# equinor/gordo-components

Measured on NVIDIA H100. Metric: anomaly windows/sec (64-tag feedforward_hourglass AE, 1k machines x 10k rows per GPU, fused predict+score), higher is better.
Workload: dtype split tf32/bf16/fp16

## Files before the change

### gordo_components_b200/csrc/ffae_infer_tc.cu

```cuda
#include <atomic>
#include <cuda_bf16.h>
#include <cuda_fp16.h>
#include "gb_common.cuh"
#include "gb_sm90.cuh"

namespace {

using namespace gb::sm90;

constexpr int TILE = 64;
constexpr int NWG = 3;
constexpr int NTHREADS = 128 * NWG;
constexpr int MAXL = 8;
constexpr int W = 64;
constexpr int BOX_COLS = 32;
constexpr int BOX_BYTES = TILE * BOX_COLS * 4;
constexpr int TILE_BYTES = 2 * BOX_BYTES;
constexpr int STAGE_BYTES = 2 * TILE_BYTES * NWG;
constexpr int OBOX_ROWS = 16;
constexpr int OBOX_BYTES = OBOX_ROWS * BOX_COLS * 4;

struct TcArgs {
  CUtensorMap tm_x, tm_y;
  CUtensorMap tm_o[4];
  int T;
  int L;
  int N[MAXL], Np[MAXL], k16[MAXL];
  int img0_ofs[MAXL], img1_ofs[MAXL], img2_ofs[MAXL];
  int bias_ofs[MAXL];
  int pofs[MAXL];
  int K[MAXL];
  int w_bytes;
  int vec_ofs;
  int stage_ofs;
  int n_jobs, tiles_per_job;
  long pstride;
  const float* params;
  const gb_job* jobs;
  const float *y, *scale, *feat_thr, *agg_thr;
  float *o_model, *o_ts, *o_tu, *o_conf, *o_tots, *o_totu, *o_totconf;
  unsigned int* work_ctr;
};

constexpr float TANH_ARG_SCALE = 2.8853900817779268f;
__device__ __forceinline__ float tanh_from_scaled(float t) {
  float e, r;
  asm("ex2.approx.ftz.f32 %0, %1;" : "=f"(e) : "f"(t));
  asm("rcp.approx.ftz.f32 %0, %1;" : "=f"(r) : "f"(e + 1.0f));
  return fmaf(-2.0f, r, 1.0f);
}

__device__ __forceinline__ uint32_t pack_bf16(float lo, float hi) {
  const __nv_bfloat162 p = __floats2bfloat162_rn(lo, hi);
  return *reinterpret_cast<const uint32_t*>(&p);
}
__device__ __forceinline__ float trunc_tf32(float v) { return __uint_as_float(__float_as_uint(v) & 0xffffe000u); }
__device__ __forceinline__ void split_f16(float a0, float a1, uint32_t& w1, uint32_t& w2) {
  const __half2 h = __floats2half2_rn(a0, a1);
  const float2 f = __half22float2(h);
  const __half2 r = __floats2half2_rn(a0 - f.x, a1 - f.y);
  w1 = *reinterpret_cast<const uint32_t*>(&h);
  w2 = *reinterpret_cast<const uint32_t*>(&r);
}

__host__ __device__ __forceinline__ int tf32_row(int k) { return (k & ~7) | (((k & 7) >> 1) + 4 * (k & 1)); }

template <int N>
__device__ __forceinline__ void mma_layer0(float* d, const uint32_t (&xhi)[4][8], const uint32_t (&alo)[4][4], const uint32_t (&abf)[4][4],
                                           uint32_t img0, uint32_t img1, uint32_t img2, int k16) {
  const uint32_t lbo = N * 16, step = 2 * N * 16;
#pragma unroll
  for (int ks = 0; ks < 8; ++ks)
    if (ks < 2 * k16) {
      const uint32_t a[4] = {xhi[ks >> 1][4 * (ks & 1) + 0], xhi[ks >> 1][4 * (ks & 1) + 1], xhi[ks >> 1][4 * (ks & 1) + 2], xhi[ks >> 1][4 * (ks & 1) + 3]};
      if (N == 16) wgmma_rs_tf32_n16(d, a, desc_noswizzle(img0 + ks * step, lbo, 128), ks > 0);
      if (N == 32) wgmma_rs_tf32_n32(d, a, desc_noswizzle(img0 + ks * step, lbo, 128), ks > 0);
      if (N == 48) wgmma_rs_tf32_n48(d, a, desc_noswizzle(img0 + ks * step, lbo, 128), ks > 0);
      if (N == 64) wgmma_rs_tf32_n64(d, a, desc_noswizzle(img0 + ks * step, lbo, 128), ks > 0);
    }
#pragma unroll
  for (int ks = 0; ks < 4; ++ks)
    if (ks < k16) {
      if (N == 16) wgmma_rs_bf16_n16(d, alo[ks], desc_noswizzle(img1 + ks * step, lbo, 128), 1);
      if (N == 32) wgmma_rs_bf16_n32(d, alo[ks], desc_noswizzle(img1 + ks * step, lbo, 128), 1);
      if (N == 48) wgmma_rs_bf16_n48(d, alo[ks], desc_noswizzle(img1 + ks * step, lbo, 128), 1);
      if (N == 64) wgmma_rs_bf16_n64(d, alo[ks], desc_noswizzle(img1 + ks * step, lbo, 128), 1);
    }
#pragma unroll
  for (int ks = 0; ks < 4; ++ks)
    if (ks < k16) {
      if (N == 16) wgmma_rs_bf16_n16(d, abf[ks], desc_noswizzle(img2 + ks * step, lbo, 128), 1);
      if (N == 32) wgmma_rs_bf16_n32(d, abf[ks], desc_noswizzle(img2 + ks * step, lbo, 128), 1);
      if (N == 48) wgmma_rs_bf16_n48(d, abf[ks], desc_noswizzle(img2 + ks * step, lbo, 128), 1);
      if (N == 64) wgmma_rs_bf16_n64(d, abf[ks], desc_noswizzle(img2 + ks * step, lbo, 128), 1);
    }
}
template <int N>
__device__ __forceinline__ void mma_f16(float* d, const uint32_t* a, uint64_t desc, uint32_t acc) {
  if (N == 16) wgmma_rs_f16_n16(d, a, desc, acc);
  if (N == 32) wgmma_rs_f16_n32(d, a, desc, acc);
  if (N == 48) wgmma_rs_f16_n48(d, a, desc, acc);
  if (N == 64) wgmma_rs_f16_n64(d, a, desc, acc);
}
template <int N>
__device__ __forceinline__ void mma_hidden(float* d, const uint32_t (&a1)[4][4], const uint32_t (&a2)[4][4], uint32_t img0, uint32_t img1, int k16) {
  const uint32_t lbo = N * 16, step = 2 * N * 16;
#pragma unroll
  for (int ks = 0; ks < 4; ++ks)
    if (ks < k16) mma_f16<N>(d, a2[ks], desc_noswizzle(img0 + ks * step, lbo, 128), ks > 0);
#pragma unroll
  for (int ks = 0; ks < 4; ++ks)
    if (ks < k16) mma_f16<N>(d, a1[ks], desc_noswizzle(img1 + ks * step, lbo, 128), 1);
#pragma unroll
  for (int ks = 0; ks < 4; ++ks)
    if (ks < k16) mma_f16<N>(d, a1[ks], desc_noswizzle(img0 + ks * step, lbo, 128), 1);
}

__device__ __forceinline__ int box_ofs(int r, int col) { return r * 128 + (((col >> 2) ^ (r & 7)) << 4) + ((col & 3) << 2); }
__device__ __forceinline__ int tile_ofs(int r, int col) { return (col >> 5) * BOX_BYTES + box_ofs(r, col & 31); }

__device__ __forceinline__ void warpgroup_sync(int wg) { asm volatile("bar.sync %0, 128;" ::"r"(wg + 1) : "memory"); }

__device__ __forceinline__ void fence_acc(float (&d)[32]) {
#pragma unroll
  for (int i = 0; i < 32; ++i) fence_reg(d[i]);
}
template <int R, int C>
__device__ __forceinline__ void fence_frag(uint32_t (&f)[R][C]) {
#pragma unroll
  for (int i = 0; i < R; ++i)
#pragma unroll
    for (int j = 0; j < C; ++j) fence_reg(f[i][j]);
}

__global__ void __launch_bounds__(NTHREADS, 1) ffae_tc_kernel(const __grid_constant__ TcArgs a) {
  extern __shared__ __align__(1024) uint8_t smem[];
  const int tid = threadIdx.x, lane = tid & 31;
  const int warp = __shfl_sync(0xffffffffu, tid >> 5, 0);
  const int wg = warp >> 2, wq = warp & 3;
  const int g = lane >> 2, t = lane & 3;
  const uint32_t sbase = smem_u32(smem);
  const int TP = a.T, L = a.L;
  const bool has_y = a.y != nullptr;
  const bool totals = has_y && (a.o_tots || a.o_totu || a.o_totconf);
  const float inv_w = 1.0f / (float)TP;

  __shared__ __align__(8) unsigned long long s_bar[2 * NWG];
  const uint32_t stage = (sbase + a.stage_ofs + 1023) & ~1023u;
  const uint32_t xbuf = stage + wg * 2 * TILE_BYTES, ybuf = xbuf + TILE_BYTES;
  const uint8_t* xs = smem + (xbuf - sbase);
  const uint8_t* ys = smem + (ybuf - sbase);
  const uint32_t bar_x = smem_u32(&s_bar[wg]), bar_y = smem_u32(&s_bar[NWG + wg]);
  const bool leader = (tid & 127) == 0;
  uint32_t x_phase = 0, y_phase = 0;
  const uint32_t obox0 = ybuf + wq * OBOX_BYTES, obox1 = obox0 + BOX_BYTES;
  if (tid == 0) {
    for (int i = 0; i < 2 * NWG; ++i) mbar_init(smem_u32(&s_bar[i]), 1);
    asm volatile("fence.mbarrier_init.release.cluster;" ::: "memory");
  }

  __shared__ int s_item[3];
  __shared__ int s_range[2];
  if (tid == 0) s_range[0] = s_range[1] = 0;
  int cur_slot = -1;

  while (true) {
    if (tid == 0) {
      const int tpj = a.tiles_per_job, g_total = a.n_jobs * tpj;
      int gg = s_range[0], g_end = s_range[1];
      if (gg >= g_end) {
        const int seen = (int)*reinterpret_cast<volatile unsigned int*>(a.work_ctr);
        const int left = g_total - seen, per_cta = left / (int)gridDim.x;
        int size = per_cta * 2 >= 3 * tpj ? tpj : (per_cta >= tpj / 3 ? (tpj + 2) / 3 : (tpj + 5) / 6);
        if (size < 1) size = 1;
        if (seen % tpj != 0 && size > tpj - seen % tpj) size = tpj - seen % tpj;
        gg = (int)atomicAdd(a.work_ctr, (unsigned int)size);
        g_end = gg + size < g_total ? gg + size : g_total;
      }
      if (gg >= g_total) {
        s_item[0] = -1;
      } else {
        const int job_id = gg / tpj, tile_begin = gg - job_id * tpj;
        const int tile_end = min(tpj, tile_begin + (g_end - gg));
        s_item[0] = job_id; s_item[1] = tile_begin; s_item[2] = tile_end;
        gg += tile_end - tile_begin;
      }
      s_range[0] = gg; s_range[1] = g_end;
    }
    __syncthreads();
    const int job_id = s_item[0], tile_begin = s_item[1], tile_end = s_item[2];
    if (job_id < 0) break;
    const gb_job job = a.jobs[job_id];
    const int row_begin = tile_begin * TILE;
    if (row_begin >= job.n_rows) {
      __syncthreads();
      continue;
    }
    const int row_end = min(job.n_rows, tile_end * TILE);
    const int n_tiles = (row_end - row_begin + TILE - 1) / TILE;

    if (job.slot != cur_slot) {
      cur_slot = job.slot;
      const float* P = a.params + (long)job.slot * a.pstride;
      for (int i = tid; i < a.w_bytes / 16; i += NTHREADS) reinterpret_cast<uint4*>(smem)[i] = make_uint4(0, 0, 0, 0);
      __syncthreads();
      for (int l = 0; l < L; ++l) {
        const int K = a.K[l], N = a.N[l], Np = a.Np[l], KN = K * N;
        const float* Ws = P + a.pofs[l];
        for (int i = tid; i < KN; i += NTHREADS) {
          const int k = i / N, n = i - k * N;
          const float w = __ldg(Ws + i);
          const int i8 = ((k >> 3) * Np + n) * 8 + (k & 7);
          if (l == 0) {
            const float hi = __uint_as_float((__float_as_uint(w) + 0x1000u) & 0xffffe000u);
            const int kt = tf32_row(k);
            reinterpret_cast<float*>(smem + a.img0_ofs[0])[((kt >> 2) * Np + n) * 4 + (kt & 3)] = hi;
            reinterpret_cast<__nv_bfloat16*>(smem + a.img1_ofs[0])[i8] = __float2bfloat16_rn(hi);
            reinterpret_cast<__nv_bfloat16*>(smem + a.img2_ofs[0])[i8] = __float2bfloat16_rn(w - hi);
          } else {
            const __half w1 = __float2half_rn(w);
            reinterpret_cast<__half*>(smem + a.img0_ofs[l])[i8] = w1;
            reinterpret_cast<__half*>(smem + a.img1_ofs[l])[i8] = __float2half_rn(w - __half2float(w1));
          }
        }
        const float bscale = (l + 1 < L) ? TANH_ARG_SCALE : 1.0f;
        for (int n = tid; n < N; n += NTHREADS) reinterpret_cast<float*>(smem + a.bias_ofs[l])[n] = __ldg(Ws + KN + n) * bscale;
      }
      float* vec = reinterpret_cast<float*>(smem + a.vec_ofs);
      if (tid < W) {
        vec[tid] = (tid < TP && a.scale) ? __ldg(a.scale + (long)job.slot * TP + tid) : 0.f;
        vec[W + tid] = (tid < TP && a.feat_thr) ? 1.0f / __ldg(a.feat_thr + (long)job.slot * TP + tid) : 0.f;
      }
      fence_proxy_async();
    }
    __syncthreads();

    const float* vec = reinterpret_cast<const float*>(smem + a.vec_ofs);
    auto load_tile = [&](const CUtensorMap* m, uint32_t buf, uint32_t bar, int tt) {
      const int row = (int)(job.x_row + row_begin + tt * TILE);
      mbar_expect_tx(bar, TILE_BYTES);
      tma_load_2d(buf, m, 0, row, bar);
      tma_load_2d(buf + BOX_BYTES, m, BOX_COLS, row, bar);
    };
    if (leader && wg < n_tiles) load_tile(&a.tm_x, xbuf, bar_x, wg);
    for (int tt = wg; tt < n_tiles; tt += NWG) {
      float d[32];
      uint32_t a1[4][4] = {}, a2[4][4] = {};
      {
        float xr[2][16];
        mbar_wait(bar_x, x_phase);
        x_phase ^= 1;
#pragma unroll
        for (int hr = 0; hr < 2; ++hr)
#pragma unroll
          for (int c = 0; c < 8; ++c) {
            const float2 v = *reinterpret_cast<const float2*>(xs + tile_ofs(wq * 16 + g + 8 * hr, 8 * c + 2 * t));
            xr[hr][2 * c] = v.x;
            xr[hr][2 * c + 1] = v.y;
          }
        if (lane == 0) bulk_wait_read<0>();
        warpgroup_sync(wg);
        if (leader) {
          if (tt + NWG < n_tiles) load_tile(&a.tm_x, xbuf, bar_x, tt + NWG);
          if (has_y) load_tile(&a.tm_y, ybuf, bar_y, tt);
        }
        uint32_t xhi[4][8], alo[4][4], abf[4][4];
#pragma unroll
        for (int kk = 0; kk < 4; ++kk) {
#pragma unroll
          for (int hh = 0; hh < 2; ++hh) {
            xhi[kk][4 * hh + 0] = __float_as_uint(trunc_tf32(xr[0][4 * kk + 2 * hh]));
            xhi[kk][4 * hh + 1] = __float_as_uint(trunc_tf32(xr[1][4 * kk + 2 * hh]));
            xhi[kk][4 * hh + 2] = __float_as_uint(trunc_tf32(xr[0][4 * kk + 2 * hh + 1]));
            xhi[kk][4 * hh + 3] = __float_as_uint(trunc_tf32(xr[1][4 * kk + 2 * hh + 1]));
          }
#pragma unroll
          for (int q = 0; q < 4; ++q) {
            const float v0 = xr[q & 1][4 * kk + 2 * (q >> 1)], v1 = xr[q & 1][4 * kk + 2 * (q >> 1) + 1];
            alo[kk][q] = pack_bf16(v0 - trunc_tf32(v0), v1 - trunc_tf32(v1));
            abf[kk][q] = pack_bf16(v0, v1);
          }
        }
        const int k16 = a.k16[0];
        const uint32_t i0 = sbase + a.img0_ofs[0], i1 = sbase + a.img1_ofs[0], i2 = sbase + a.img2_ofs[0];
        wgmma_fence();
        switch (a.Np[0]) {
          case 16: mma_layer0<16>(d, xhi, alo, abf, i0, i1, i2, k16); break;
          case 32: mma_layer0<32>(d, xhi, alo, abf, i0, i1, i2, k16); break;
          case 48: mma_layer0<48>(d, xhi, alo, abf, i0, i1, i2, k16); break;
          default: mma_layer0<64>(d, xhi, alo, abf, i0, i1, i2, k16); break;
        }
        wgmma_commit();
        wgmma_wait<0>();
        fence_acc(d);
        fence_frag(xhi);
        fence_frag(alo);
        fence_frag(abf);
      }

      for (int l = 0; l < L; ++l) {
        if (l > 0) {
          const uint32_t i0 = sbase + a.img0_ofs[l], i1 = sbase + a.img1_ofs[l];
          const int k16 = a.k16[l];
          wgmma_fence();
          switch (a.Np[l]) {
            case 16: mma_hidden<16>(d, a1, a2, i0, i1, k16); break;
            case 32: mma_hidden<32>(d, a1, a2, i0, i1, k16); break;
            case 48: mma_hidden<48>(d, a1, a2, i0, i1, k16); break;
            default: mma_hidden<64>(d, a1, a2, i0, i1, k16); break;
          }
          wgmma_commit();
          wgmma_wait<0>();
          fence_acc(d);
          fence_frag(a1);
          fence_frag(a2);
        }
        if (l + 1 == L) break;
        const float* bl = reinterpret_cast<const float*>(smem + a.bias_ofs[l]);
        const int nt = a.Np[l] >> 3;
#pragma unroll
        for (int j = 0; j < 8; ++j) {
          if (j < nt) {
            const float2 b = *reinterpret_cast<const float2*>(bl + 8 * j + 2 * t);
            const float v0 = tanh_from_scaled(fmaf(d[4 * j], TANH_ARG_SCALE, b.x)), v1 = tanh_from_scaled(fmaf(d[4 * j + 1], TANH_ARG_SCALE, b.y));
            const float v2 = tanh_from_scaled(fmaf(d[4 * j + 2], TANH_ARG_SCALE, b.x)), v3 = tanh_from_scaled(fmaf(d[4 * j + 3], TANH_ARG_SCALE, b.y));
            split_f16(v0, v1, a1[j >> 1][2 * (j & 1)], a2[j >> 1][2 * (j & 1)]);
            split_f16(v2, v3, a1[j >> 1][2 * (j & 1) + 1], a2[j >> 1][2 * (j & 1) + 1]);
          }
        }
      }

      const float* bo = reinterpret_cast<const float*>(smem + a.bias_ofs[L - 1]);
      const int wrow = row_begin + tt * TILE + wq * 16;
      const int trow = wrow + g;
      const int nt = a.Np[L - 1] >> 3;
      float2 yr[2][8];
      if (has_y) {
        mbar_wait(bar_y, y_phase);
        y_phase ^= 1;
#pragma unroll
        for (int hr = 0; hr < 2; ++hr)
#pragma unroll
          for (int j = 0; j < 8; ++j) yr[hr][j] = *reinterpret_cast<const float2*>(ys + tile_ofs(wq * 16 + g + 8 * hr, 8 * j + 2 * t));
      }
      auto model_out = [&](int hr, int j) {
        const float2 b = *reinterpret_cast<const float2*>(bo + 8 * j + 2 * t);
        return j < nt ? make_float2(d[4 * j + 2 * hr] + b.x, d[4 * j + 2 * hr + 1] + b.y) : make_float2(0.f, 0.f);
      };

      const int n_live = min(row_end - wrow, OBOX_ROWS);
      if (n_live > 0) {
        int k = 0;
#pragma unroll
        for (int arr = 0; arr < 4; ++arr) {
          float* o = arr == 0 ? a.o_model : arr == 1 ? a.o_tu : arr == 2 ? a.o_ts : a.o_conf;
          if (o == nullptr || (arr > 0 && !has_y)) continue;
#pragma unroll
          for (int h = 0; h < 2; ++h) {
            if (h == 1 && TP <= BOX_COLS) break;
            const uint32_t box = (k & 1) ? obox1 : obox0;
            if (k >= 2 && lane == 0) bulk_wait_read<1>();
            __syncwarp();
            uint8_t* bs = smem + (box - sbase);
#pragma unroll
            for (int hr = 0; hr < 2; ++hr)
#pragma unroll
              for (int jj = 0; jj < 4; ++jj) {
                const int j = 4 * h + jj, col = 8 * j + 2 * t;
                float2 v = model_out(hr, j);
                if (arr > 0) {
                  const float2 yv = yr[hr][j];
                  v = make_float2(fabsf(v.x - yv.x), fabsf(v.y - yv.y));
                  const float2 s = *reinterpret_cast<const float2*>(vec + (arr == 3 ? W : 0) + col);
                  if (arr > 1) v = make_float2(v.x * s.x, v.y * s.y);
                }
                *reinterpret_cast<float2*>(bs + box_ofs(g + 8 * hr, 8 * jj + 2 * t)) = v;
              }
            fence_proxy_async();
            __syncwarp();
            if (n_live == OBOX_ROWS) {
              if (lane == 0) {
                tma_store_2d(&a.tm_o[arr], box, BOX_COLS * h, (int)(job.out_row + wrow));
                bulk_commit();
              }
            } else {
              const int cols = min(BOX_COLS, TP - BOX_COLS * h);
              for (int i = lane; i < n_live * 8; i += 32) {
                const int r = i >> 3, c = i & 7;
                if (4 * c < cols)
                  __stcs(reinterpret_cast<float4*>(o + (job.out_row + wrow + r) * (long)TP + BOX_COLS * h + 4 * c),
                         *reinterpret_cast<const float4*>(bs + box_ofs(r, 4 * c)));
              }
            }
            ++k;
          }
        }
      }
      if (totals) {
        float ss[2] = {0.f, 0.f}, su[2] = {0.f, 0.f};
#pragma unroll
        for (int hr = 0; hr < 2; ++hr)
#pragma unroll
          for (int j = 0; j < 8; ++j) {
            const int col = 8 * j + 2 * t;
            if (j < nt && col < TP) {
              const float2 yh = model_out(hr, j), yv = yr[hr][j];
              const float2 sc = *reinterpret_cast<const float2*>(vec + col);
              const float2 df = make_float2(fabsf(yh.x - yv.x), fabsf(yh.y - yv.y));
              const float2 e = make_float2(df.x * sc.x, df.y * sc.y);
              su[hr] += df.x * df.x + df.y * df.y;
              ss[hr] += e.x * e.x + e.y * e.y;
            }
          }
#pragma unroll
        for (int hr = 0; hr < 2; ++hr) {
          ss[hr] += __shfl_xor_sync(0xffffffffu, ss[hr], 1);
          ss[hr] += __shfl_xor_sync(0xffffffffu, ss[hr], 2);
          su[hr] += __shfl_xor_sync(0xffffffffu, su[hr], 1);
          su[hr] += __shfl_xor_sync(0xffffffffu, su[hr], 2);
          const int r = trow + 8 * hr;
          if (t == 0 && r < row_end) {
            const long go = job.out_row + r;
            const float ts_ = ss[hr] * inv_w, tu_ = su[hr] * inv_w;
            if (a.o_tots) a.o_tots[go] = ts_;
            if (a.o_totu) a.o_totu[go] = tu_;
            if (a.o_totconf) a.o_totconf[go] = ts_ / __ldg(a.agg_thr + job.slot);
          }
        }
      }
    }
    __syncthreads();
  }
  if (lane == 0) bulk_wait<0>();
}

constexpr int WORK_CTRS = 1024;
__device__ unsigned int g_work_ctr[WORK_CTRS];

int plan_smem(const gb_ffnet* net, TcArgs& a) {
  const int L = net->n_layers;
  a.L = L;
  a.T = net->dims[0];
  int ofs = 0, pofs = 0;
  for (int l = 0; l < L; ++l) {
    a.K[l] = net->dims[l];
    a.N[l] = net->dims[l + 1];
    a.Np[l] = gb::round_up(a.N[l], 16);
    a.k16[l] = gb::round_up(a.K[l], 16) / 16;
    a.pofs[l] = pofs;
    pofs += a.K[l] * a.N[l] + a.N[l];
    const int kp = a.k16[l] * 16;
    a.img0_ofs[l] = ofs;
    ofs += kp * a.Np[l] * (l == 0 ? 4 : 2);
    a.img1_ofs[l] = ofs;
    ofs += kp * a.Np[l] * 2;
    if (l == 0) {
      a.img2_ofs[l] = ofs;
      ofs += kp * a.Np[l] * 2;
    }
  }
  for (int l = 0; l < L; ++l) {
    a.bias_ofs[l] = ofs;
    ofs += W * 4;
  }
  a.w_bytes = gb::round_up(ofs, 16);
  ofs = a.w_bytes;
  a.vec_ofs = ofs; ofs += 2 * W * 4;
  a.stage_ofs = ofs; ofs += 1024 + STAGE_BYTES;
  return ofs;
}

}

extern "C" int gb_ffae_tc_supported(const gb_ffnet* net) {
  if (gb::validate_ffnet(net) != GB_OK) return GB_E_SHAPE;
  const int L = net->n_layers;
  if (L < 2 || L > MAXL || net->dims[0] != net->dims[L] || net->dims[0] > W || net->dims[0] < 24 || (net->dims[0] & 3)) {
    gb::set_error("tensor-core variant covers autoencoders of 24..%d tags (a multiple of 4) with at most %d layers", W, MAXL);
    return GB_E_SHAPE;
  }
  for (int l = 1; l < L; ++l)
    if (net->dims[l] > W) {
      gb::set_error("tensor-core variant needs hidden widths <= %d", W);
      return GB_E_SHAPE;
    }
  for (int l = 0; l < L; ++l)
    if (net->act[l] != (l + 1 < L ? GB_ACT_TANH : GB_ACT_LINEAR)) {
      gb::set_error("tensor-core variant is specialised for tanh hidden layers and a linear output (the factory defaults)");
      return GB_E_SHAPE;
    }
  TcArgs a{};
  const int smem = plan_smem(net, a);
  if (smem > 227 * 1024) {
    gb::set_error("tensor-core variant: the weights and x / y tiles of this stack need %d bytes of shared memory (227 KB per SM)", smem);
    return GB_E_SHAPE;
  }
  return GB_OK;
}

extern "C" int gb_ffae_infer_score_tc(const gb_ffnet* net, const float* params, const gb_job* jobs, int32_t n_jobs, int32_t max_rows,
                                      int64_t n_x_rows, int64_t n_out_rows, const float* x, const float* y, const float* scale,
                                      const float* feat_thr, const float* agg_thr, float* out_model, float* out_tag_scaled,
                                      float* out_tag_unscaled, float* out_total_scaled, float* out_total_unscaled, float* out_conf,
                                      float* out_total_conf, int32_t flags, void* stream) {
  int rc = gb_ffae_tc_supported(net);
  if (rc != GB_OK) return rc;
  GB_REQUIRE(flags == 0, GB_E_ARG, "variant bits above the low byte must be 0");
  GB_REQUIRE(n_x_rows > 0 && n_out_rows > 0, GB_E_ARG, "the tensor-core variant needs the row counts of x and of the outputs");
  TcArgs a{};
  const size_t smem = (size_t)plan_smem(net, a);
  GB_REQUIRE(n_x_rows < (1L << 31), GB_E_ARG, "%ld rows of x: TMA row coordinates are 32-bit", (long)n_x_rows);
  GB_REQUIRE(n_out_rows < (1L << 31), GB_E_ARG, "%ld output rows: TMA row coordinates are 32-bit", (long)n_out_rows);
  {
    CUresult r = gb::sm90::encode_map_2d(&a.tm_x, CU_TENSOR_MAP_DATA_TYPE_FLOAT32, 4, x, n_x_rows, a.T, BOX_COLS, TILE);
    if (r == CUDA_SUCCESS && y) r = gb::sm90::encode_map_2d(&a.tm_y, CU_TENSOR_MAP_DATA_TYPE_FLOAT32, 4, y, n_x_rows, a.T, BOX_COLS, TILE);
    float* const outs[4] = {out_model, out_tag_unscaled, out_tag_scaled, out_conf};
    for (int i = 0; i < 4; ++i)
      if (r == CUDA_SUCCESS && outs[i]) r = gb::sm90::encode_map_2d(&a.tm_o[i], CU_TENSOR_MAP_DATA_TYPE_FLOAT32, 4, outs[i], n_out_rows, a.T, BOX_COLS, OBOX_ROWS);
    GB_REQUIRE(r != CUDA_ERROR_NOT_FOUND, GB_E_CUDA, "cuTensorMapEncodeTiled is not available from the driver");
    GB_REQUIRE(r == CUDA_SUCCESS, GB_E_CUDA, "cuTensorMapEncodeTiled (x / y / outputs) failed with CUresult %d", (int)r);
  }

  int dev = 0, sms = 132;
  GB_CUDA_CHECK(cudaGetDevice(&dev));
  GB_CUDA_CHECK(cudaDeviceGetAttribute(&sms, cudaDevAttrMultiProcessorCount, dev));
  const int tiles_per_job = (max_rows + TILE - 1) / TILE;
  a.tiles_per_job = tiles_per_job;
  a.n_jobs = n_jobs;
  a.pstride = (long)gb_ffnet_param_stride(net);
  a.params = params; a.jobs = jobs; a.y = y; a.scale = scale; a.feat_thr = feat_thr; a.agg_thr = agg_thr;
  a.o_model = out_model; a.o_ts = out_tag_scaled; a.o_tu = out_tag_unscaled; a.o_conf = out_conf;
  a.o_tots = out_total_scaled; a.o_totu = out_total_unscaled; a.o_totconf = out_total_conf;

  const long g_total = (long)n_jobs * tiles_per_job;
  GB_REQUIRE(g_total < (1L << 31), GB_E_ARG, "%ld tiles in one launch: split the fleet", g_total);
  const int grid = (int)(g_total < sms ? g_total : sms);
  {
    static std::atomic<unsigned> next_ctr{0};
    void* base = nullptr;
    GB_CUDA_CHECK(cudaGetSymbolAddress(&base, g_work_ctr));
    a.work_ctr = static_cast<unsigned int*>(base) + (next_ctr.fetch_add(1) % WORK_CTRS);
    GB_CUDA_CHECK(cudaMemsetAsync(a.work_ctr, 0, sizeof(unsigned int), (cudaStream_t)stream));
  }
  GB_CUDA_CHECK(cudaFuncSetAttribute(ffae_tc_kernel, cudaFuncAttributeMaxDynamicSharedMemorySize, (int)smem));
  ffae_tc_kernel<<<grid, NTHREADS, smem, (cudaStream_t)stream>>>(a);
  GB_CUDA_CHECK(cudaGetLastError());
  return GB_OK;
}
```

Baseline: 1.607 billion.

## Prefetch layer weights into registers and issue first tile TMA before restaging

When a block switches to a new machine's parameters, it now loads each layer's weights and bias into a register batch, prefetching the next layer's batch while converting the current one. Previously each layer did serial strided global loads. The first input tile's TMA load is also issued before the weight restage, so the load overlaps the restage. This adds register pressure (22 floats per thread) and assumes a layer's weights and bias fit in one batch. That assumption is enforced by a static_assert for 64-wide layers.

```diff
diff --git a/gordo_components_b200/csrc/ffae_infer_tc.cu b/gordo_components_b200/csrc/ffae_infer_tc.cu
--- a/gordo_components_b200/csrc/ffae_infer_tc.cu
+++ b/gordo_components_b200/csrc/ffae_infer_tc.cu
@@ -19,6 +19,8 @@
 constexpr int STAGE_BYTES = 2 * TILE_BYTES * NWG;
 constexpr int OBOX_ROWS = 16;
 constexpr int OBOX_BYTES = OBOX_ROWS * BOX_COLS * 4;
+constexpr int RESTAGE_BATCH = 11;
+static_assert(RESTAGE_BATCH * NTHREADS >= W * W + W, "a layer's kernel and bias are one batch of loads");
 
 struct TcArgs {
   CUtensorMap tm_x, tm_y;
@@ -199,17 +201,47 @@
     const int row_end = min(job.n_rows, tile_end * TILE);
     const int n_tiles = (row_end - row_begin + TILE - 1) / TILE;
 
+    auto load_tile = [&](const CUtensorMap* m, uint32_t buf, uint32_t bar, int tt) {
+      const int row = (int)(job.x_row + row_begin + tt * TILE);
+      mbar_expect_tx(bar, TILE_BYTES);
+      tma_load_2d(buf, m, 0, row, bar);
+      tma_load_2d(buf + BOX_BYTES, m, BOX_COLS, row, bar);
+    };
+    if (leader && wg < n_tiles) load_tile(&a.tm_x, xbuf, bar_x, wg);
+
     if (job.slot != cur_slot) {
       cur_slot = job.slot;
       const float* P = a.params + (long)job.slot * a.pstride;
+      float v[RESTAGE_BATCH], vn[RESTAGE_BATCH];
+      auto fetch = [&](float (&dst)[RESTAGE_BATCH], int l) {
+        const float* Ws = P + a.pofs[l];
+        const int n_l = a.K[l] * a.N[l] + a.N[l];
+#pragma unroll
+        for (int u = 0; u < RESTAGE_BATCH; ++u) {
+          const int i = tid + u * NTHREADS;
+          dst[u] = i < n_l ? __ldg(Ws + i) : 0.f;
+        }
+      };
+      fetch(v, 0);
+      const bool vt = tid < TP;
+      const float sc = vt && a.scale ? __ldg(a.scale + (long)job.slot * TP + tid) : 0.f;
+      const float ft = vt && a.feat_thr ? __ldg(a.feat_thr + (long)job.slot * TP + tid) : 0.f;
       for (int i = tid; i < a.w_bytes / 16; i += NTHREADS) reinterpret_cast<uint4*>(smem)[i] = make_uint4(0, 0, 0, 0);
       __syncthreads();
       for (int l = 0; l < L; ++l) {
+        if (l + 1 < L) fetch(vn, l + 1);
         const int K = a.K[l], N = a.N[l], Np = a.Np[l], KN = K * N;
-        const float* Ws = P + a.pofs[l];
-        for (int i = tid; i < KN; i += NTHREADS) {
+        const float bscale = (l + 1 < L) ? TANH_ARG_SCALE : 1.0f;
+#pragma unroll
+        for (int u = 0; u < RESTAGE_BATCH; ++u) {
+          const int i = tid + u * NTHREADS;
+          if (i >= KN + N) break;
+          if (i >= KN) {
+            reinterpret_cast<float*>(smem + a.bias_ofs[l])[i - KN] = v[u] * bscale;
+            continue;
+          }
           const int k = i / N, n = i - k * N;
-          const float w = __ldg(Ws + i);
+          const float w = v[u];
           const int i8 = ((k >> 3) * Np + n) * 8 + (k & 7);
           if (l == 0) {
             const float hi = __uint_as_float((__float_as_uint(w) + 0x1000u) & 0xffffe000u);
@@ -223,26 +255,19 @@
             reinterpret_cast<__half*>(smem + a.img1_ofs[l])[i8] = __float2half_rn(w - __half2float(w1));
           }
         }
-        const float bscale = (l + 1 < L) ? TANH_ARG_SCALE : 1.0f;
-        for (int n = tid; n < N; n += NTHREADS) reinterpret_cast<float*>(smem + a.bias_ofs[l])[n] = __ldg(Ws + KN + n) * bscale;
+#pragma unroll
+        for (int u = 0; u < RESTAGE_BATCH; ++u) v[u] = vn[u];
       }
       float* vec = reinterpret_cast<float*>(smem + a.vec_ofs);
       if (tid < W) {
-        vec[tid] = (tid < TP && a.scale) ? __ldg(a.scale + (long)job.slot * TP + tid) : 0.f;
-        vec[W + tid] = (tid < TP && a.feat_thr) ? 1.0f / __ldg(a.feat_thr + (long)job.slot * TP + tid) : 0.f;
+        vec[tid] = sc;
+        vec[W + tid] = vt && a.feat_thr ? 1.0f / ft : 0.f;
       }
       fence_proxy_async();
     }
     __syncthreads();
 
     const float* vec = reinterpret_cast<const float*>(smem + a.vec_ofs);
-    auto load_tile = [&](const CUtensorMap* m, uint32_t buf, uint32_t bar, int tt) {
-      const int row = (int)(job.x_row + row_begin + tt * TILE);
-      mbar_expect_tx(bar, TILE_BYTES);
-      tma_load_2d(buf, m, 0, row, bar);
-      tma_load_2d(buf + BOX_BYTES, m, BOX_COLS, row, bar);
-    };
-    if (leader && wg < n_tiles) load_tile(&a.tm_x, xbuf, bar_x, wg);
     for (int tt = wg; tt < n_tiles; tt += NWG) {
       float d[32];
       uint32_t a1[4][4] = {}, a2[4][4] = {};
```

Result: faster. 1.656 billion, median of 6 (+3.1%).
